# FeggieBoss/raytracing-course

Measured on NVIDIA B200. Metric: Mpaths/s, higher is better.
Workload: dtype f32

## Files before the change

include/rtc_b200.h:

```cpp
#ifndef RTC_B200_H
#define RTC_B200_H
#include <stdint.h>
#ifdef __cplusplus
extern "C" {
#endif

typedef struct rtc_scene rtc_scene;

typedef enum {
    RTC_OK = 0,
    RTC_ERR_IO = -1,
    RTC_ERR_NO_DEVICE = -2,
    RTC_ERR_CUDA = -3,
    RTC_ERR_ARG = -4,
    RTC_ERR_UNSUPPORTED = -5
} rtc_status;

#define RTC_TRAVERSAL_INDEX   0
#define RTC_TRAVERSAL_REFTREE 1

const char* rtc_last_error(void);
int rtc_version(void);
int rtc_device_count(void);

// ... 23 lines not shown
int rtc_intersect(const rtc_scene* s, long n, const float* o_host, const float* d_host,
                  int32_t* id_host, float* t_host, float* normal_host, int32_t* interior_host, int mode);
int rtc_intersect_dev(rtc_scene* s, long n, const float* o_dev, const float* d_dev, int32_t* id_dev, float* t_dev,
                      float* normal_dev, int32_t* interior_dev, int mode, void* stream);
int rtc_primitive_intersect(const rtc_scene* s, int prim, long n, const float* o_host, const float* d_host,
                            int32_t* hit_host, float* t_host, float* normal_host, int32_t* interior_host);
int rtc_camera_rays(const rtc_scene* s, long n, const float* xy_host, float* o_host, float* d_host);
int rtc_mix_pdf(const rtc_scene* s, long n, const float* x_host, const float* nrm_host, const float* d_host,
                float* pdf_host);
int rtc_mix_sample(const rtc_scene* s, long n, const float* x_host, const float* nrm_host,
                   uint32_t seed, uint32_t sample, uint32_t bounce, float* dir_host);
int rtc_tonemap_u8(const rtc_scene* s, long npix, const float* rgb_host, uint8_t* out_host);

int rtc_render_accumulate(rtc_scene* s, uint32_t seed, uint32_t sample_begin, uint32_t sample_count,
                          float* accum_dev, void* stream);
int rtc_render_counters(rtc_scene* s, void* stream, uint64_t out[8]);
int rtc_render_reset_counters(rtc_scene* s);
int rtc_traverse_lanes(rtc_scene* s, void* stream, uint64_t out[8]);
int rtc_render_resolve(rtc_scene* s, const float* accum_dev, uint32_t total_samples, uint8_t* rgb_dev, void* stream);
int rtc_render_u8(rtc_scene* s, uint32_t seed, uint8_t* rgb_host);
int rtc_render_sum(rtc_scene* s, uint32_t seed, uint32_t sample_begin, uint32_t sample_count, float* sum_host);
int rtc_render_ppm(rtc_scene* s, uint32_t seed, const char* out_path);
#define RTC_ADAPTIVE_TILE 8
int rtc_render_adaptive(rtc_scene* s, uint32_t seed, float tolerance, uint32_t min_samples, uint32_t max_samples,
                        uint8_t* rgb_host, float* halves_host, uint32_t* spp_host, uint64_t stats[4]);
int rtc_render_u8_multi(rtc_scene* s, const int* devices, int ndev, uint32_t seed, uint8_t* rgb_host, float* sum_host);
int rtc_render_ppm_multi(rtc_scene* s, const int* devices, int ndev, uint32_t seed, const char* out_path);
int rtc_render_adaptive_multi(rtc_scene* s, const int* devices, int ndev, uint32_t seed, float tolerance, uint32_t min_samples,
                              uint32_t max_samples, uint8_t* rgb_host, float* halves_host, uint32_t* spp_host, uint64_t stats[4]);
int rtc_denoise(rtc_scene* s, const float* halves_host, const uint32_t* spp_host, float strength, uint8_t* rgb_host, float* mean_host);
int rtc_render_denoised(rtc_scene* s, uint32_t seed, float tolerance, uint32_t min_samples, uint32_t max_samples, float strength,
// ... 20 lines not shown
```

raytracing-course_b200/__init__.py:

```python
import ctypes as C
import os

import numpy as np

HERE = os.path.dirname(os.path.abspath(__file__))
LIB_PATH = os.path.join(HERE, "librtc_b200.so")
CLI_PATH = os.path.join(HERE, "raytracing_hw5")
HEADER_PATH = os.path.join(os.path.dirname(HERE), "include", "rtc_b200.h")

TRAVERSAL_INDEX = 0
TRAVERSAL_REFTREE = 1
DENOISE_STRENGTH = 0.45

_f32 = np.ctypeslib.ndpointer(dtype=np.float32, flags="C_CONTIGUOUS")
_i32 = np.ctypeslib.ndpointer(dtype=np.int32, flags="C_CONTIGUOUS")
_u32 = np.ctypeslib.ndpointer(dtype=np.uint32, flags="C_CONTIGUOUS")
_u64 = np.ctypeslib.ndpointer(dtype=np.uint64, flags="C_CONTIGUOUS")
_u8 = np.ctypeslib.ndpointer(dtype=np.uint8, flags="C_CONTIGUOUS")

_SIGNATURES = {
    "rtc_last_error": (C.c_char_p, []),
    "rtc_version": (C.c_int, []),
    "rtc_device_count": (C.c_int, []),
    "rtc_scene_load": (C.c_void_p, [C.c_char_p, C.c_int]),
# ... 345 lines not shown
                                                    C.c_void_p(t_ptr), C.c_void_p(normal_ptr), C.c_void_p(interior_ptr),
                                                    mode, C.c_void_p(stream or 0)))

    def RenderPPM(self, path, seed=0):
        _check(self.lib, self.lib.rtc_render_ppm(self.h, seed, os.fsencode(path)))

    def render_accumulate(self, accum_ptr, seed, sample_begin, sample_count, stream=None):
        _check(self.lib, self.lib.rtc_render_accumulate(self.h, seed, sample_begin, sample_count,
                                                         C.c_void_p(accum_ptr), C.c_void_p(stream or 0)))

    def render_resolve(self, accum_ptr, total_samples, rgb_ptr, stream=None):
        _check(self.lib, self.lib.rtc_render_resolve(self.h, C.c_void_p(accum_ptr), total_samples,
                                                      C.c_void_p(rgb_ptr), C.c_void_p(stream or 0)))

    def counters(self, stream=None):
        out = np.zeros(8, np.uint64)
        _check(self.lib, self.lib.rtc_render_counters(self.h, C.c_void_p(stream or 0), out))
        keys = ["paths", "rays", "launches", "batches", "index_node_visits", "fallback_rays", "prim_tests", "traversed_rays"]
        return dict(zip(keys, [int(v) for v in out[:8]]))

    def traverse_lanes(self, stream=None):
        out = np.zeros(8, np.uint64)
        _check(self.lib, self.lib.rtc_traverse_lanes(self.h, C.c_void_p(stream or 0), out))
        kinds = ["visit", "leaf", "finish", "refill"]
        return {k: {"iterations": int(out[i]), "lanes": (float(out[4 + i]) / float(out[i]) if out[i] else 0.0)}
                for i, k in enumerate(kinds)}

    def set_profiling(self, kernel_events=False, count_visits=False):
        _check(self.lib, self.lib.rtc_set_profiling(self.h, int(kernel_events), int(count_visits)))

    def profile(self, stream=None, reset=True):
        ms = np.zeros(4, np.float64)
        n = np.zeros(4, np.uint64)
        _check(self.lib, self.lib.rtc_render_profile(self.h, C.c_void_p(stream or 0), ms, n, int(reset)))
# ... 18 lines not shown
```

raytracing-course_b200/csrc/bvh_build.cpp:

```cpp
#include <algorithm>
#include <chrono>
#include <cstdio>
#include <cstdlib>
#include <cmath>
#include <cstring>
#include <future>
#include <thread>
#include <numeric>
#include <stdexcept>

#include "scene_host.h"

namespace rtc {

static const float kInf = 1e18f;

static Aabb empty_box() { return Aabb{{kInf, kInf, kInf}, {-kInf, -kInf, -kInf}}; }
static void grow(Aabb& b, vec3 p) {
    b.mx.x = std::max(b.mx.x, p.x); b.mn.x = std::min(b.mn.x, p.x);
    b.mx.y = std::max(b.mx.y, p.y); b.mn.y = std::min(b.mn.y, p.y);
    b.mx.z = std::max(b.mx.z, p.z); b.mn.z = std::min(b.mn.z, p.z);
}
static void grow(Aabb& b, const Aabb& o) { grow(b, o.mx); grow(b, o.mn); }
static float surface(const Aabb& b) {
// ... 444 lines not shown
    std::memcpy(&r.w, &bits, 4);
    return r;
}

namespace {
struct PhaseTimer {
    bool on = std::getenv("RTC_TIMING") != nullptr;
    std::chrono::steady_clock::time_point t0 = std::chrono::steady_clock::now();
    void lap(const char* what) {
        if (!on) return;
        auto t1 = std::chrono::steady_clock::now();
        std::fprintf(stderr, "[rtc timing] %-28s %8.1f ms\n", what, std::chrono::duration<double, std::milli>(t1 - t0).count());
        t0 = t1;
    }
};
}

void HostScene::init() {
    PhaseTimer timer;
    const uint32_t n = (uint32_t)prims.size();
    if (n >= IREF_MAX_PRIMS) throw std::runtime_error("scene has more than 2^24 primitives");

    std::vector<Primitive> original = prims;
    std::vector<int32_t> perm(n);
    std::iota(perm.begin(), perm.end(), 0);
    const Primitive* P = original.data();
    nbvh = (uint32_t)(std::partition(perm.begin(), perm.end(), [P](int32_t i) { return P[i].type != PT_PLANE; }) - perm.begin());

    nodes.clear();
    root = 0;
// ... 33 lines not shown
            vec3 nrm = normalize(cross(p.d1 - p.d0, p.d2 - p.d0));
            F.geo0[i] = f4{p.d0.x, p.d0.y, p.d0.z, nrm.x};
            F.geo1[i] = f4{p.d1.x, p.d1.y, p.d1.z, nrm.y};
            F.geo2[i] = f4{p.d2.x, p.d2.y, p.d2.z, nrm.z};
        } else {
            F.geo0[i] = f4{p.d0.x, p.d0.y, p.d0.z, 0.f};
            F.geo1[i] = f4{0, 0, 0, 0};
            F.geo2[i] = f4{0, 0, 0, 0};
        }
        F.xf_pos[i] = pack(p.pos, flags);
        F.xf_rot[i] = f4{p.rot.x, p.rot.y, p.rot.z, p.rot.w};
        F.mat0[i] = pack(p.col, (uint32_t)p.material);
        F.mat1[i] = f4{p.emission.x, p.emission.y, p.emission.z, p.ior};
    }
    F.lights = lights;
    for (const PointLight& l : point_lights) {
        vec3 nd = l.directed ? normalize(l.dir) : mk3(0, 0, 0);
        F.plights.push_back(pack(l.intensity, l.directed ? 1u : 0u));
        F.plights.push_back(pack(l.pos, 0));
        F.plights.push_back(pack(l.att, 0));
        F.plights.push_back(pack(nd, 0));
    }
    for (uint32_t i = nbvh; i < n; ++i) {
        const Primitive& p = prims[i];
        bool rot_ident = p.rot.x == 0.f && p.rot.y == 0.f && p.rot.z == 0.f && p.rot.w == 1.f;
        F.planes.push_back(pack(p.d0, i));
        F.planes.push_back(pack(p.pos, rot_ident ? 1u : 0u));
    }

    timer.lap("flatten primitives");
// ... 88 lines not shown
```

raytracing-course_b200/csrc/c_api.cu:

```cuda
#include <cuda_runtime.h>

#include <algorithm>
#include <array>
#include <cfloat>
#include <cmath>
#include <chrono>
#include <cstdio>
#include <cstdlib>
#include <cstring>
#include <fstream>
#include <functional>
#include <map>
#include <memory>
#include <sstream>
#include <stdexcept>
#include <string>
#include <thread>
#include <vector>

#include "device_scene.h"
#include "rt_kernels.h"
#include "rtc_b200.h"
#include "scene_host.h"

// ... 42 lines not shown
    Handle() = default;
    Handle(Handle&& o) noexcept : h(o.h) { o.h = nullptr; }
    ~Handle() { if (h) destroy(h); }
    cudaError_t ensure() { return h ? cudaSuccess : create(&h); }
    operator H() const { return h; }
};
cudaError_t new_stream(cudaStream_t* st) { return cudaStreamCreateWithFlags(st, cudaStreamNonBlocking); }
cudaError_t new_event(cudaEvent_t* e) { return cudaEventCreateWithFlags(e, cudaEventDisableTiming); }
cudaError_t new_timed_event(cudaEvent_t* e) { return cudaEventCreate(e); }
using Stream = Handle<cudaStream_t, new_stream, cudaStreamDestroy>;
using Event = Handle<cudaEvent_t, new_event, cudaEventDestroy>;
using TimedEvent = Handle<cudaEvent_t, new_timed_event, cudaEventDestroy>;

constexpr uint64_t kDefaultBatchPaths = 1ull << 24;
constexpr int kMaxDepthSlots = 64;
constexpr int kStatWords = 16;
constexpr int kMaxWhittedDepth = 32;
}

struct rtc_scene {
    std::shared_ptr<HostScene> host_ptr;
    HostScene& host;
    rtc_scene() : host_ptr(std::make_shared<HostScene>()), host(*host_ptr) {}
    explicit rtc_scene(const std::shared_ptr<HostScene>& h) : host_ptr(h), host(*h) {}
    int device = -1;
    int sms = 0;
    int traversal = RTC_TRAVERSAL_INDEX;
    uint64_t batch_paths = kDefaultBatchPaths;
    uint64_t device_bytes = 0;
    DevBuf<unsigned char> arena_dev[2];
    PinnedBuf<unsigned char> arena_host;
// ... 420 lines not shown
        if (l.stream) {
            cudaError_t e = cudaStreamSynchronize(l.stream);
            if (e != cudaSuccess) return e;
        }
    return cudaSuccess;
}

int ensure_wavefront(rtc_scene* s, uint64_t cap, int nlanes) {
    for (int i = 0; i < nlanes; ++i) {
        rtc_scene::Lane& l = s->lanes[i];
        CU(l.stream.ensure());
        CU(l.done.ensure());
        for (auto& set : l.path) for (auto& b : set) CU(b.ensure(cap));
        for (auto& b : l.hit_id) CU(b.ensure(cap));
        CU(l.trav_queue.ensure(cap * kTraverseQueueWords));
        CU(l.queue.ensure(4 * kMaxDepthSlots));
    }
    return RTC_OK;
}

struct PathMap {
    const uint32_t* plist;
    uint32_t npix;
    uint32_t sample_first;
};
int fork_lanes(rtc_scene* s, cudaStream_t user) {
    CU(s->fork.ensure());
    CU(cudaEventRecord(s->fork, user));
    return RTC_OK;
}
int join_lanes(rtc_scene* s, unsigned used, cudaStream_t user) {
// ... 17 lines not shown
    const int nlanes = s->profiling ? 1 : whole ? s->nlanes : (int)(nbatches < (uint64_t)s->nlanes ? nbatches : (uint64_t)s->nlanes);
    const int lane_first = whole ? (int)(s->next_lane++ % (unsigned)s->nlanes) : 0;
    if ((rc = ensure_wavefront(s, cap, nlanes))) return rc;
    for (int i = 0; i < nlanes; ++i)
        if (!whole || i == lane_first) {
            CU(cudaStreamWaitEvent(s->lanes[i].stream, s->fork, 0));
            *used |= 1u << i;
        }
    uint64_t batch = 0;
    for (uint64_t first = 0; first < total; first += cap, ++batch) {
        rtc_scene::Lane& L = s->lanes[(lane_first + batch) % nlanes];
        cudaStream_t st = L.stream;
        LaunchCtx c{st, s->sms};
        uint32_t* tqc = L.queue.p + 2 * kMaxDepthSlots;
        uint32_t* cursor = L.queue.p + 3 * kMaxDepthSlots;
        uint32_t count = (uint32_t)((total - first) < cap ? (total - first) : cap);
        CU(cudaMemsetAsync(L.queue.p, 0, 4 * kMaxDepthSlots * sizeof(uint32_t), st));
        PathSoA cur{L.path[0][0].p, L.path[0][1].p, L.path[0][2].p};
        PathSoA nxt{L.path[1][0].p, L.path[1][1].p, L.path[1][2].p};
        HitSoA hcur{L.hit_id[0].p}, hnxt{L.hit_id[1].p};
        s->span_begin(0, st);
        if (map.plist) launch_generate_list(c, S, cur, hcur, L.queue.p, L.trav_queue.p, tqc, first, count, seed, map.plist, map.npix, map.sample_first);
        else launch_generate(c, S, cur, hcur, L.queue.p, L.trav_queue.p, tqc, first, count, seed, map.sample_first);
        s->span_end(st);
        s->launches++;
        for (uint32_t b = 1; b <= depth; ++b) {
            s->span_begin(1, st);
            if (s->traversal == RTC_TRAVERSAL_REFTREE) launch_extend_reftree(c, S, cur, hcur, L.queue.p + 2 * (b - 1), count);
            else launch_traverse(c, S, cur, hcur, count, L.trav_queue.p, tqc + (b - 1), cursor + (b - 1), s->count_visits, s->stats.p);
            s->span_end(st);
            s->span_begin(2, st);
            launch_shade(c, S, cur, hcur, nxt, hnxt, L.queue.p + 2 * (b - 1), L.queue.p + 2 * b, L.trav_queue.p, tqc + b, count,
                         target, b, seed);
            s->span_end(st);
            s->launches += 2;
            PathSoA tmp = cur; cur = nxt; nxt = tmp;
            HitSoA htmp = hcur; hcur = hnxt; hnxt = htmp;
        }
        launch_tally(c, L.queue.p, tqc, depth, s->stats.p);
        s->launches++;
    }
    return RTC_OK;
}

}

extern "C" {

const char* rtc_last_error(void) { return g_error.c_str(); }
int rtc_version(void) { return 100; }
int rtc_device_count(void) {
    int n = 0;
    if (cudaGetDeviceCount(&n) != cudaSuccess) { cudaGetLastError(); return 0; }
    return n;
// ... 279 lines not shown
    CU(accum4.ensure(npix));
    CU(cudaStreamWaitEvent(user, s->accum4_idle[a4], 0));
    CU(cudaMemsetAsync(accum4.p, 0, npix * sizeof(float4), user));
    if ((rc = arena_begin(s, user, &S))) return rc;
    if ((rc = fork_lanes(s, user))) return rc;
    unsigned used = 0;
    if ((rc = render_paths(s, S, seed, PathMap{nullptr, (uint32_t)npix, sample_begin}, total, accum4.p, &used))) return rc;
    if ((rc = join_lanes(s, used, user))) return rc;
    launch_fold(LaunchCtx{user, s->sms}, accum4.p, accum_dev, (uint32_t)npix);
    s->launches++;
    CU(cudaEventRecord(s->accum4_idle[a4], user));
    if ((rc = arena_end(s, user))) return rc;
    CU(cudaGetLastError());
    return RTC_OK;
}
int rtc_render_counters(rtc_scene* s, void* stream, uint64_t out[8]) {
    int rc = need_device(s);
    if (rc) return rc;
    if (!out) return fail(RTC_ERR_ARG, "null argument");
    CU(cudaStreamSynchronize((cudaStream_t)stream));
    CU(sync_lanes(s));
    unsigned long long h[8];
    CU(cudaMemcpy(h, s->stats.p, sizeof h, cudaMemcpyDeviceToHost));
    for (int i = 0; i < 8; ++i) out[i] = h[i];
    out[2] = s->launches;
    return RTC_OK;
}
int rtc_traverse_lanes(rtc_scene* s, void* stream, uint64_t out[8]) {
    int rc = need_device(s);
    if (rc) return rc;
    if (!out) return fail(RTC_ERR_ARG, "null argument");
    CU(cudaStreamSynchronize((cudaStream_t)stream));
    CU(sync_lanes(s));
    unsigned long long h[8];
    CU(cudaMemcpy(h, s->stats.p + 8, sizeof h, cudaMemcpyDeviceToHost));
    for (int i = 0; i < 8; ++i) out[i] = h[i];
    return RTC_OK;
}
int rtc_render_reset_counters(rtc_scene* s) {
    int rc = need_device(s);
// ... 672 lines not shown
```

raytracing-course_b200/csrc/device_scene.h:

```cpp
#pragma once
#include <cuda_runtime.h>
#include <math.h>
#include <stdint.h>
#include <string.h>

#include "scene_host.h"

namespace rtc {

struct DevScene {
    const float4* geo0;
    const float4* geo1;
    const float4* geo2;
    const float4* xf_pos;
    const float4* xf_rot;
    const float4* mat0;
    const float4* mat1;
    const float4* inodes;
    const float4* rnodes;
    const uint4* rmeta;
    const uint32_t* lca;
    const int32_t* lights;
    const float4* ubox;
    const float4* planes;
    const float4* plights;

    uint32_t nprims, nbvh, nnodes, root, iroot, lca_levels, nlights, ref_depth;
    uint32_t iroot_ref[4];
    uint32_t width, height, ray_depth, nplanes;
    float3 cam_pos, cam_right, cam_up, cam_forward;
    float tan_fov_x, tan_fov_y;
    float3 bg;
    uint32_t dialect, nplights;
    uint32_t features;
    float eps;
    float plane_tmax;
    float3 ambient;
};

inline void fill_dev_scalars(const HostScene& host, DevScene& S) {
    S.nplanes = (uint32_t)(host.flat.planes.size() / 2);
    S.nprims = (uint32_t)host.prims.size(); S.nbvh = host.nbvh; S.nnodes = (uint32_t)host.nodes.size();
    S.root = host.root; S.iroot = host.flat.iroot; S.lca_levels = host.flat.lca_levels;
    for (int c = 0; c < 4; ++c) S.iroot_ref[c] = IREF_NONE;
    if (host.flat.iroot != IREF_NONE && !(host.flat.iroot & IREF_LEAF)) {
        const f4& refs = host.flat.inodes[kIndexNodeF4 * (size_t)(host.flat.iroot & IREF_NODE_MASK) + 3];
        memcpy(S.iroot_ref, &refs, sizeof S.iroot_ref);
    }
    S.nlights = (uint32_t)host.lights.size(); S.ref_depth = host.flat.ref_depth;
    S.width = host.cam.width; S.height = host.cam.height; S.ray_depth = host.ray_depth;
    S.cam_pos = make_float3(host.cam.pos.x, host.cam.pos.y, host.cam.pos.z);
    S.cam_right = make_float3(host.cam.right.x, host.cam.right.y, host.cam.right.z);
    S.cam_up = make_float3(host.cam.up.x, host.cam.up.y, host.cam.up.z);
    S.cam_forward = make_float3(host.cam.forward.x, host.cam.forward.y, host.cam.forward.z);
    float tx = (float)tan((double)(host.cam.fov_x / 2));
    S.tan_fov_x = tx;
    S.tan_fov_y = tx * (float)host.cam.height / (float)host.cam.width;
    S.bg = make_float3(host.background.x, host.background.y, host.background.z);
    S.nplights = (uint32_t)host.point_lights.size();
    S.dialect = (uint32_t)host.dialect;
    S.features = host.flat.features;
    S.eps = host.dialect <= DIALECT_HW3 ? 1e-3f : 1e-4f;
    S.plane_tmax = host.dialect <= DIALECT_HW3 ? 3.0e38f : 1e5f;
    S.ambient = make_float3(host.ambient.x, host.ambient.y, host.ambient.z);
}

struct PathSoA {
    float4* o;
    float4* d;
    float4* beta;
};
struct HitSoA {
    uint32_t* id;
};

constexpr uint32_t HIT_MISS = 0xFFFFFFFFu;
constexpr uint32_t HIT_INTERIOR = 1u << 30;

}
// ... 1 lines not shown
```

raytracing-course_b200/csrc/rt_device.cuh:

```cuda
#pragma once
#include <cuda_fp16.h>
#include <cuda_runtime.h>
#include <math_constants.h>
#include <stdint.h>

#include "device_scene.h"
#include "scene_host.h"
#include "vecmath.h"

namespace rtc {

#define RT_D __device__ __forceinline__
#ifdef __CUDACC__
#define RT_D_COLD static __device__ __noinline__
#else
#define RT_D_COLD static inline
#endif

constexpr float kInfF = 1e18f;
constexpr float kPi = 3.14159274101257324f;
constexpr int kRejectCap = 64;
constexpr int kMaxRecords = 24;
constexpr int kIndexStack = 64;
constexpr int kRefStack = 96;
// ... 583 lines not shown
        if (!(FEAT & FE_ROTATION) || __float_as_uint(b.w)) {
            vec3 n = ld3(a);
            t = -dot(o - ld3(b), n) / dot(d, n);
            ok = t > 0.f && !(t > S.plane_tmax);
        } else {
            vec3 lo = o, ld = d;
            to_local(S, prim, prim_flags(S, prim), lo, ld);
            Isect is;
            ok = isect_plane(lo, ld, ld3(a), S.plane_tmax, is);
            t = is.t;
        }
        if (ok && t < closest) { closest = t; id = (int)prim; }
    }
}

struct SceneHit {
    int id;
    float t;
    vec3 n;
    int interior;
};

template <int MODE>
RT_D SceneHit scene_intersect(const DevScene& S, vec3 o, vec3 d, uint32_t* visits, uint32_t* tests, uint32_t* fallbacks) {
    SceneHit h;
    h.id = -1; h.t = 0.f; h.n = mk3(0, 0, 0); h.interior = 0;
    float closest;
    closest_plane(S, o, d, closest, h.id);
    BestHit b;
    if (MODE == 1) {
// ... 188 lines not shown
```

raytracing-course_b200/csrc/rt_kernels.cu:

```cuda
#include <cassert>

#include "rt_device.cuh"
#include "rt_kernels.h"

namespace rtc {

static_assert(kNodeWidth == 4, "a traverse-queue entry carries the 4 root children a ray enters");
constexpr unsigned kFullMask = 0xFFFFFFFFu;
#ifndef RTC_TRAVERSE_CHUNK
#define RTC_TRAVERSE_CHUNK 64
#endif
#ifndef RTC_TRAVERSE_CHUNK_DIV
#define RTC_TRAVERSE_CHUNK_DIV 4
#endif
#ifndef RTC_TRAVERSE_CHUNK_MAX
#define RTC_TRAVERSE_CHUNK_MAX 512
#endif
constexpr uint32_t kChunk = RTC_TRAVERSE_CHUNK;

#ifndef RTC_NO_STREAM_STATE
#define WF_LD(ptr) __ldcs(ptr)
#define WF_ST(ptr, v) __stcs(ptr, v)
#else
#define WF_LD(ptr) (*(ptr))
// ... 323 lines not shown
#endif
}

#ifndef RTC_SHADE_THREADS
#define RTC_SHADE_THREADS 128
#endif
#ifndef RTC_SHADE_MIN_BLOCKS_FULL
#define RTC_SHADE_MIN_BLOCKS_FULL 6
#endif
#ifndef RTC_SHADE_MIN_BLOCKS_LEAN
#define RTC_SHADE_MIN_BLOCKS_LEAN 9
#endif
template <bool HW3, uint32_t FEAT>
__global__ void __launch_bounds__(RTC_SHADE_THREADS, (FEAT & (FE_ROTATION | FE_ELLIPSOID)) ? RTC_SHADE_MIN_BLOCKS_FULL : RTC_SHADE_MIN_BLOCKS_LEAN) k_shade(DevScene S, PathSoA P, HitSoA H, PathSoA N, HitSoA HN, const uint32_t* qin,
                                                uint32_t* qout, uint32_t* tq, uint32_t* tq_count, float4* accum4, uint32_t bounce,
                                                uint32_t seed, uint32_t cap) {
    const QueueView view = queue_view(qin);
    const uint32_t lane = threadIdx.x & 31;
    const float eps = S.eps;
    const bool sorted_in = bounce > 1 && !HW3;
    const bool sort_out = !HW3 && S.nlights != 0 && bounce + 1 < S.ray_depth;
    for (uint32_t at = blockIdx.x * blockDim.x + threadIdx.x; at < view.total; at += gridDim.x * blockDim.x) {
        bool alive = false;
        vec3 no = mk3(0, 0, 0), nd = mk3(0, 0, 0), beta = mk3(0, 0, 0);
        uint32_t pixel = 0, sample = 0;
        uint32_t i; bool back;
        if (queue_slot(view, at, cap, i, back)) {
            const float4 b4 = WF_LD(P.beta + i), o4 = WF_LD(P.o + i);
            beta = ld3(b4);
            pixel = __float_as_uint(b4.w); sample = __float_as_uint(o4.w);
            uint32_t prim = WF_LD(H.id + i);
            Isect is;
            vec3 o = ld3(o4), d = ld3(WF_LD(P.d + i));
            vec3 L;
            float4 xp = make_float4(0.f, 0.f, 0.f, 0.f), g0 = xp, g1 = xp, g2 = xp, m0 = xp, m1 = xp;
            if (prim != HIT_MISS) {
// ... 57 lines not shown
                            vec3 rd = reflect_dir(normal, nd_in);
                            no = p + eps * rd; nd = rd;
                        } else {
                            float cos2 = sqrtf(1.f - sin2 * sin2);
                            float e = eta1 / eta2;
                            vec3 fr = e * (-dir) + (e * dn - cos2) * normal;
                            no = p + eps * fr; nd = fr;
                            if (!interior) beta = beta * col;
                        }
                        alive = true;
                    }
                }
            }
            if (L.x != 0.f || L.y != 0.f || L.z != 0.f) deposit(accum4, pixel, L);
        }
        unsigned mask = __ballot_sync(kFullMask, alive);
        if (mask) {
            const uint32_t lt = (1u << lane) - 1u;
            bool to_back = false;
            if (sort_out && alive) to_back = mix_picks_light(S, Rng{seed, pixel, sample, bounce + 1});
            const unsigned bmask = __ballot_sync(kFullMask, to_back), fmask = mask & ~bmask;
            unsigned long long both = 0;
            uint32_t tbase = 0;
            if (lane == 0) both = atomicAdd(reinterpret_cast<unsigned long long*>(qout),
                                            (unsigned long long)__popc(fmask) | ((unsigned long long)__popc(bmask) << 32));
            float cd = 0.f;
            uint32_t id = HIT_MISS, enters = 0;
            if (alive) enters = pre_step<FEAT>(S, no, nd, cd, id);
            const unsigned emask = __ballot_sync(kFullMask, enters != 0);
            if (emask && lane == 0) tbase = atomicAdd(tq_count, (uint32_t)__popc(emask));
            both = __shfl_sync(kFullMask, both, 0);
            const uint32_t dst = to_back ? cap - 1u - ((uint32_t)(both >> 32) + __popc(bmask & lt))
                                         : (uint32_t)both + __popc(fmask & lt);
            if (alive) {
                WF_ST(N.o + dst, make_float4(no.x, no.y, no.z, __uint_as_float(sample)));
                WF_ST(N.d + dst, make_float4(nd.x, nd.y, nd.z, cd));
                WF_ST(N.beta + dst, make_float4(beta.x, beta.y, beta.z, __uint_as_float(pixel)));
                WF_ST(HN.id + dst, id);
            }
            if (emask) {
                tbase = __shfl_sync(kFullMask, tbase, 0);
                if (enters) tq_store(tq, tbase + __popc(emask & lt), dst | (enters << kTqSlotBits), no, nd, cd);
            }
        }
    }
}

__global__ void k_tally(const uint32_t* q, const uint32_t* tqc, uint32_t ray_depth, unsigned long long* stats) {
    unsigned long long rays = 0, queued = 0;
    for (uint32_t b = 0; b < ray_depth; ++b) { rays += q[2 * b] + q[2 * b + 1]; queued += tqc[b]; }
    atomicAdd(stats + 0, (unsigned long long)q[0]);
    atomicAdd(stats + 1, rays);
    atomicAdd(stats + 3, 1ull);
    atomicAdd(stats + 7, queued);
}

RT_D float aces(float x) {
    const float a = 2.51f, b = 0.03f, c = 2.43f, d = 0.59f, e = 0.14f;
    float num = __fmul_rn(x, __fadd_rn(__fmul_rn(a, x), b));
    float den = __fadd_rn(__fmul_rn(x, __fadd_rn(__fmul_rn(c, x), d)), e);
    float y = __fdiv_rn(num, den);
    y = (y < 1.f) ? y : 1.f;
    y = (y < 0.f) ? 0.f : y;
    return y;
}
// ... 385 lines not shown
    }
    return cache[slot][dev];
}
void launch_traverse(const LaunchCtx& c, const DevScene& S, PathSoA P, HitSoA H, uint32_t max_count, const uint32_t* tq,
                     const uint32_t* tq_count, uint32_t* cursor, bool count_visits, unsigned long long* stats) {
    const int per_sm = count_visits ? resident_blocks(k_traverse<true>, 1) : resident_blocks(k_traverse<false>, 0);
    int grid = grid_for((uint64_t)max_count, 128, c.sms, per_sm);
    if (count_visits) k_traverse<true><<<grid, 128, 0, c.stream>>>(S, P, H, tq, tq_count, cursor, stats);
    else k_traverse<false><<<grid, 128, 0, c.stream>>>(S, P, H, tq, tq_count, cursor, stats);
}
void launch_extend_reftree(const LaunchCtx& c, const DevScene& S, PathSoA P, HitSoA H, const uint32_t* q, uint32_t cap) {
    k_extend_reftree<<<grid_for(cap, 128, c.sms, 16), 128, 0, c.stream>>>(S, P, H, q, cap);
}
void launch_shade(const LaunchCtx& c, const DevScene& S, PathSoA P, HitSoA H, PathSoA N, HitSoA HN, const uint32_t* qin,
                  uint32_t* qout, uint32_t* tq, uint32_t* tq_count, uint32_t max_count, float4* accum4, uint32_t bounce,
                  uint32_t seed) {
    const int grid = grid_for(max_count, RTC_SHADE_THREADS, c.sms, 2048 / RTC_SHADE_THREADS);
#define RTC_SHADE(HW3, FEAT) k_shade<HW3, FEAT><<<grid, RTC_SHADE_THREADS, 0, c.stream>>>(S, P, H, N, HN, qin, qout, tq, tq_count, accum4, bounce, seed, max_count)
#ifdef RTC_SHADE_NO_SPECIALISATION
    const uint32_t feat = FE_ALL;
#else
    const uint32_t feat = S.features;
#endif
    if (S.dialect == DIALECT_HW3) RTC_SHADE(true, FE_ALL);
    else if (feat == 0) RTC_SHADE(false, 0);
    else if (feat == FE_SPECULAR) RTC_SHADE(false, FE_SPECULAR);
    else RTC_SHADE(false, FE_ALL);
#undef RTC_SHADE
}
void launch_expand_lca(const LaunchCtx& c, uint32_t* lca, const uint4* rmeta, uint32_t n, uint32_t levels) {
    for (uint32_t l = 1; l < levels; ++l)
        k_expand_lca_level<<<grid_for(n, 256, c.sms, 8), 256, 0, c.stream>>>(lca + (size_t)(l - 1) * n, lca + (size_t)l * n, rmeta, n, 1u << (l - 1));
}
void launch_expand_boxes(const LaunchCtx& c, const float4* sparse, uint32_t n, float4* ubox) {
    k_expand_boxes<<<grid_for(n, 256, c.sms, 8), 256, 0, c.stream>>>(sparse, n, ubox);
}
void launch_expand_palette(const LaunchCtx& c, const float4* palette, const uint16_t* index, uint32_t n, float4* out0, float4* out1) {
    k_expand_palette<<<grid_for(n, 256, c.sms, 8), 256, 0, c.stream>>>(palette, index, n, out0, out1);
}
void launch_fill_identity_rotations(const LaunchCtx& c, float4* rot, uint32_t n) {
    k_fill_identity_rotations<<<grid_for(n, 256, c.sms, 8), 256, 0, c.stream>>>(rot, n);
}
void launch_tally(const LaunchCtx& c, const uint32_t* q, const uint32_t* tqc, uint32_t ray_depth, unsigned long long* stats) {
    k_tally<<<1, 1, 0, c.stream>>>(q, tqc, ray_depth, stats);
}
void launch_fold(const LaunchCtx& c, const float4* accum4, float* accum, uint32_t npix) {
    k_fold<<<grid_for(npix, 256, c.sms, 8), 256, 0, c.stream>>>(accum4, accum, npix);
}
void launch_resolve(const LaunchCtx& c, const float* accum, float inv_samples, uint32_t nvalues, uint8_t* out) {
    k_resolve<<<grid_for(nvalues, 256, c.sms, 8), 256, 0, c.stream>>>(accum, inv_samples, nvalues, out);
}
void launch_resolve_peers(const LaunchCtx& c, const PeerAccums& A, float inv_samples, uint32_t nvalues, uint8_t* out, float* sum) {
    k_resolve_peers<<<grid_for(nvalues, 256, c.sms, 8), 256, 0, c.stream>>>(A, inv_samples, nvalues, out, sum);
}
void launch_tonemap(const LaunchCtx& c, const float* rgb, uint32_t nvalues, uint8_t* out) {
    k_tonemap<<<grid_for(nvalues, 256, c.sms, 8), 256, 0, c.stream>>>(rgb, nvalues, out);
}
void launch_pack_rays(const LaunchCtx& c, long n, const float* o, const float* d, PathSoA P, uint32_t* q) {
    k_pack_rays<<<grid_for((uint64_t)n, 256, c.sms, 8), 256, 0, c.stream>>>(n, o, d, P, q);
// ... 22 lines not shown
```

raytracing-course_b200/csrc/rt_kernels.h:

```cpp
#pragma once
#include <cuda_runtime.h>
#include <stdint.h>

#include "device_scene.h"

namespace rtc {

constexpr uint32_t kTraverseQueueWords = 8;

struct LaunchCtx {
    cudaStream_t stream;
    int sms;
};

void launch_generate(const LaunchCtx& c, const DevScene& S, PathSoA P, HitSoA H, uint32_t* q, uint32_t* tq, uint32_t* tq_count,
                     uint64_t first_path, uint32_t count, uint32_t seed, uint32_t sample_begin);
void launch_generate_list(const LaunchCtx& c, const DevScene& S, PathSoA P, HitSoA H, uint32_t* q, uint32_t* tq, uint32_t* tq_count,
                          uint64_t first_path, uint32_t count, uint32_t seed, const uint32_t* plist, uint32_t npix, uint32_t sample_first);
constexpr uint32_t kAdaptiveTile = 8;
static_assert(kAdaptiveTile * kAdaptiveTile == 64, "k_adaptive_tiles: one warp per tile, two pixels per lane");
enum { ADAPTIVE_FIRST = 0, ADAPTIVE_DECIDE = 1, ADAPTIVE_LAST = 2 };
void launch_adaptive_tiles(const LaunchCtx& c, const float4* A, const float4* B, uint32_t width, uint32_t height,
                           const uint32_t* tiles_in, uint32_t ntiles, uint32_t n, float inv_a, float inv_b, float tau, int mode,
                           uint32_t* tile_n, uint32_t* tiles_out, uint32_t* pixels_out, uint32_t* counts_out, uint32_t shard,
// ... 3 lines not shown
constexpr int kDenoiseRadius = 7, kDenoisePatch = 3, kDenoiseVarRadius = 1;
constexpr float kDenoiseAlpha = 1.f, kDenoiseEps = 1e-8f;
constexpr int kDenoiseTileW = 32, kDenoiseTileH = 16;
constexpr int kDenoiseApron = kDenoiseRadius + kDenoisePatch + kDenoiseVarRadius;
void launch_denoise_prep(const LaunchCtx& c, const float* halves, const uint32_t* spp, uint32_t npix, float* u, float4* D, float4* V,
                         uint8_t* rgb);
cudaError_t launch_denoise_nlm(const LaunchCtx& c, const float* u, const float4* D, const float4* V, uint32_t width, uint32_t height,
                               uint32_t tile_row0, uint32_t tile_rows, uint32_t buf_row0, float k2, float* mean, uint8_t* rgb);
void launch_pre(const LaunchCtx& c, const DevScene& S, PathSoA P, HitSoA H, const uint32_t* qcount, uint32_t max_count,
                uint32_t* tq, uint32_t* tq_count);
void launch_traverse(const LaunchCtx& c, const DevScene& S, PathSoA P, HitSoA H, uint32_t max_count, const uint32_t* tq,
                     const uint32_t* tq_count, uint32_t* cursor, bool count_visits, unsigned long long* stats);
void launch_extend_reftree(const LaunchCtx& c, const DevScene& S, PathSoA P, HitSoA H, const uint32_t* q, uint32_t cap);
void launch_shade(const LaunchCtx& c, const DevScene& S, PathSoA P, HitSoA H, PathSoA N, HitSoA HN, const uint32_t* qin,
                  uint32_t* qout, uint32_t* tq, uint32_t* tq_count, uint32_t max_count, float4* accum4, uint32_t bounce,
                  uint32_t seed);
void launch_fold(const LaunchCtx& c, const float4* accum4, float* accum, uint32_t npix);
void launch_expand_lca(const LaunchCtx& c, uint32_t* lca, const uint4* rmeta, uint32_t n, uint32_t levels);
void launch_expand_boxes(const LaunchCtx& c, const float4* sparse, uint32_t n, float4* ubox);
void launch_fill_identity_rotations(const LaunchCtx& c, float4* rot, uint32_t n);
void launch_expand_palette(const LaunchCtx& c, const float4* palette, const uint16_t* index, uint32_t n, float4* out0, float4* out1);
void launch_tally(const LaunchCtx& c, const uint32_t* q, const uint32_t* tqc, uint32_t ray_depth, unsigned long long* stats);
void launch_resolve(const LaunchCtx& c, const float* accum, float inv_samples, uint32_t nvalues, uint8_t* out);
void launch_tonemap(const LaunchCtx& c, const float* rgb, uint32_t nvalues, uint8_t* out);
constexpr int kMaxPeers = 16;
struct PeerAccums {
    const float* p[kMaxPeers];
    int n;
};
void launch_resolve_peers(const LaunchCtx& c, const PeerAccums& A, float inv_samples, uint32_t nvalues, uint8_t* out, float* sum);
struct PeerHalves {
    const float4* a[kMaxPeers];
    const float4* b[kMaxPeers];
    const uint32_t* tile_n[kMaxPeers];
    int n;
};
void launch_resolve_adaptive_peers(const LaunchCtx& c, const PeerHalves& P, uint32_t width, uint32_t npix, uint8_t* out, float* halves,
// ... 19 lines not shown
```

raytracing-course_b200/csrc/scene_host.h:

```cpp
#pragma once
#include <cstdint>
#include <string>
#include <vector>

#include "vecmath.h"

#ifndef RTC_NODE_CONES
#define RTC_NODE_CONES 1
#endif
#ifndef RTC_NODE_CENTRE_HALF
#define RTC_NODE_CENTRE_HALF 1
#endif

namespace rtc {

enum Dialect : int {
    DIALECT_HW1 = 1,
    DIALECT_HW2 = 2,
    DIALECT_HW3 = 3,
    DIALECT_HW4 = 4,
    DIALECT_HW5 = 5
};

struct PointLight {
// ... 54 lines not shown
    std::vector<f4> xf_pos;
    std::vector<f4> xf_rot;
    std::vector<f4> mat0, mat1;
    std::vector<f4> inodes;
    uint32_t iroot = 0;
    std::vector<f4> rnodes;
    std::vector<u4> rmeta;
    std::vector<uint32_t> lca;
    uint32_t lca_levels = 0;
    std::vector<f4> ubox;
    std::vector<f4> planes;
    std::vector<int32_t> lights;
    std::vector<f4> plights;
    uint32_t index_depth = 0, ref_depth = 0, units = 0;
    uint32_t features = 0;
};

struct HostScene {
    int dialect = DIALECT_HW5;
    Camera cam;
    vec3 background{0, 0, 0};
    vec3 ambient{0, 0, 0};
    std::vector<PointLight> point_lights;
    unsigned ray_depth = 0, samples = 0;
    std::vector<Primitive> prims;
    uint32_t nbvh = 0;
    std::vector<RefNode> nodes;
    uint32_t root = 0;
    std::vector<int32_t> lights;
    FlatScene flat;

// ... 23 lines not shown
```

Before: 2047.

## Retire final-bounce rays that cannot reach emitters and early-miss rays in shade

Computes conservative world-space AABBs for emissive boxes and ellipsoids on the host and stores them in the device scene. On the last bounce, the shade kernel drops rays whose direction misses every emitter box, since they cannot add radiance. Rays that pre_step already shows miss the scene are resolved in place with the background contribution and never reach the traversal queue. New counters track retired rays. This saves traversal and shading work in exchange for extra per-ray box tests and an added atomic per warp; scenes with other emitter types or more than eight emitters turn the final-bounce cull off.

```diff
diff --git a/include/rtc_b200.h b/include/rtc_b200.h
--- a/include/rtc_b200.h
+++ b/include/rtc_b200.h
@@ -61,7 +61,7 @@
 
 int rtc_render_accumulate(rtc_scene* s, uint32_t seed, uint32_t sample_begin, uint32_t sample_count,
                           float* accum_dev, void* stream);
-int rtc_render_counters(rtc_scene* s, void* stream, uint64_t out[8]);
+int rtc_render_counters(rtc_scene* s, void* stream, uint64_t out[10]);
 int rtc_render_reset_counters(rtc_scene* s);
 int rtc_traverse_lanes(rtc_scene* s, void* stream, uint64_t out[8]);
 int rtc_render_resolve(rtc_scene* s, const float* accum_dev, uint32_t total_samples, uint8_t* rgb_dev, void* stream);
diff --git a/raytracing-course_b200/__init__.py b/raytracing-course_b200/__init__.py
--- a/raytracing-course_b200/__init__.py
+++ b/raytracing-course_b200/__init__.py
@@ -383,10 +383,11 @@
                                                       C.c_void_p(rgb_ptr), C.c_void_p(stream or 0)))
 
     def counters(self, stream=None):
-        out = np.zeros(8, np.uint64)
+        out = np.zeros(10, np.uint64)
         _check(self.lib, self.lib.rtc_render_counters(self.h, C.c_void_p(stream or 0), out))
-        keys = ["paths", "rays", "launches", "batches", "index_node_visits", "fallback_rays", "prim_tests", "traversed_rays"]
-        return dict(zip(keys, [int(v) for v in out[:8]]))
+        keys = ["paths", "rays", "launches", "batches", "index_node_visits", "fallback_rays", "prim_tests", "traversed_rays",
+                "retired_rays", "retired_final_rays"]
+        return dict(zip(keys, [int(v) for v in out]))
 
     def traverse_lanes(self, stream=None):
         out = np.zeros(8, np.uint64)
diff --git a/raytracing-course_b200/csrc/bvh_build.cpp b/raytracing-course_b200/csrc/bvh_build.cpp
--- a/raytracing-course_b200/csrc/bvh_build.cpp
+++ b/raytracing-course_b200/csrc/bvh_build.cpp
@@ -482,6 +482,55 @@
         t0 = t1;
     }
 };
+bool emitter_boxes(const HostScene& h, std::vector<f4>& out) {
+    out.clear();
+    double extent = std::max({std::fabs((double)h.cam.pos.x), std::fabs((double)h.cam.pos.y), std::fabs((double)h.cam.pos.z)});
+    if (h.nbvh) {
+        const Aabb& r = h.nodes[h.root].box;
+        extent = std::max({extent, std::fabs((double)r.mn.x), std::fabs((double)r.mn.y), std::fabs((double)r.mn.z),
+                           std::fabs((double)r.mx.x), std::fabs((double)r.mx.y), std::fabs((double)r.mx.z)});
+    }
+    for (const Primitive& p : h.prims) {
+        if (p.emission.x == 0.f && p.emission.y == 0.f && p.emission.z == 0.f) continue;
+        if ((p.type != PT_BOX && p.type != PT_ELLIPSOID) || out.size() == 2 * kMaxEmitBoxes) { out.clear(); return false; }
+        const double qx = -(double)p.rot.x, qy = -(double)p.rot.y, qz = -(double)p.rot.z, qw = p.rot.w;
+        double M[3][3];
+        for (int c = 0; c < 3; ++c) {
+            const double v[3] = {c == 0 ? 1. : 0., c == 1 ? 1. : 0., c == 2 ? 1. : 0.};
+            const double u[3] = {qy * v[2] - qz * v[1], qz * v[0] - qx * v[2], qx * v[1] - qy * v[0]};
+            const double uu[3] = {qy * u[2] - qz * u[1], qz * u[0] - qx * u[2], qx * u[1] - qy * u[0]};
+            for (int r = 0; r < 3; ++r) M[r][c] = v[r] + 2. * (qw * u[r] + uu[r]);
+        }
+        const double det = M[0][0] * (M[1][1] * M[2][2] - M[1][2] * M[2][1]) - M[0][1] * (M[1][0] * M[2][2] - M[1][2] * M[2][0]) +
+                           M[0][2] * (M[1][0] * M[2][1] - M[1][1] * M[2][0]);
+        if (!(std::fabs(det) > 1e-9)) { out.clear(); return false; }
+        double I[3][3];
+        for (int r = 0; r < 3; ++r)
+            for (int c = 0; c < 3; ++c) {
+                const int r1 = (c + 1) % 3, r2 = (c + 2) % 3, c1 = (r + 1) % 3, c2 = (r + 2) % 3;
+                I[r][c] = (M[r1][c1] * M[r2][c2] - M[r1][c2] * M[r2][c1]) / det;
+            }
+        double lo[3] = {INFINITY, INFINITY, INFINITY}, hi[3] = {-INFINITY, -INFINITY, -INFINITY};
+        const double s[3] = {p.d0.x, p.d0.y, p.d0.z}, pos[3] = {p.pos.x, p.pos.y, p.pos.z};
+        for (int corner = 0; corner < 8; ++corner)
+            for (int r = 0; r < 3; ++r) {
+                double w = pos[r];
+                for (int c = 0; c < 3; ++c) w += I[r][c] * ((corner >> c & 1) ? s[c] : -s[c]);
+                lo[r] = std::min(lo[r], w);
+                hi[r] = std::max(hi[r], w);
+            }
+        float flo[3], fhi[3];
+        for (int r = 0; r < 3; ++r) {
+            const double pad = 1e-3 * std::max({extent, std::fabs(lo[r]), std::fabs(hi[r])});
+            flo[r] = std::nextafter((float)(lo[r] - pad), -INFINITY);
+            fhi[r] = std::nextafter((float)(hi[r] + pad), INFINITY);
+            if (!std::isfinite(flo[r]) || !std::isfinite(fhi[r])) { out.clear(); return false; }
+        }
+        out.push_back(f4{flo[0], flo[1], flo[2], 0.f});
+        out.push_back(f4{fhi[0], fhi[1], fhi[2], 0.f});
+    }
+    return true;
+}
 }
 
 void HostScene::init() {
@@ -545,6 +594,7 @@
         F.mat1[i] = f4{p.emission.x, p.emission.y, p.emission.z, p.ior};
     }
     F.lights = lights;
+    F.final_cull = emitter_boxes(*this, F.emit_boxes);
     for (const PointLight& l : point_lights) {
         vec3 nd = l.directed ? normalize(l.dir) : mk3(0, 0, 0);
         F.plights.push_back(pack(l.intensity, l.directed ? 1u : 0u));
diff --git a/raytracing-course_b200/csrc/c_api.cu b/raytracing-course_b200/csrc/c_api.cu
--- a/raytracing-course_b200/csrc/c_api.cu
+++ b/raytracing-course_b200/csrc/c_api.cu
@@ -80,7 +80,7 @@
 
 constexpr uint64_t kDefaultBatchPaths = 1ull << 24;
 constexpr int kMaxDepthSlots = 64;
-constexpr int kStatWords = 16;
+constexpr int kStatWords = 18;
 constexpr int kMaxWhittedDepth = 32;
 }
 
@@ -531,7 +531,7 @@
         for (auto& set : l.path) for (auto& b : set) CU(b.ensure(cap));
         for (auto& b : l.hit_id) CU(b.ensure(cap));
         CU(l.trav_queue.ensure(cap * kTraverseQueueWords));
-        CU(l.queue.ensure(4 * kMaxDepthSlots));
+        CU(l.queue.ensure(6 * kMaxDepthSlots));
     }
     return RTC_OK;
 }
@@ -579,8 +579,9 @@
         LaunchCtx c{st, s->sms};
         uint32_t* tqc = L.queue.p + 2 * kMaxDepthSlots;
         uint32_t* cursor = L.queue.p + 3 * kMaxDepthSlots;
+        unsigned long long* retired = reinterpret_cast<unsigned long long*>(L.queue.p + 4 * kMaxDepthSlots);
         uint32_t count = (uint32_t)((total - first) < cap ? (total - first) : cap);
-        CU(cudaMemsetAsync(L.queue.p, 0, 4 * kMaxDepthSlots * sizeof(uint32_t), st));
+        CU(cudaMemsetAsync(L.queue.p, 0, 6 * kMaxDepthSlots * sizeof(uint32_t), st));
         PathSoA cur{L.path[0][0].p, L.path[0][1].p, L.path[0][2].p};
         PathSoA nxt{L.path[1][0].p, L.path[1][1].p, L.path[1][2].p};
         HitSoA hcur{L.hit_id[0].p}, hnxt{L.hit_id[1].p};
@@ -596,13 +597,13 @@
             s->span_end(st);
             s->span_begin(2, st);
             launch_shade(c, S, cur, hcur, nxt, hnxt, L.queue.p + 2 * (b - 1), L.queue.p + 2 * b, L.trav_queue.p, tqc + b, count,
-                         target, b, seed);
+                         target, b, seed, retired + b);
             s->span_end(st);
             s->launches += 2;
             PathSoA tmp = cur; cur = nxt; nxt = tmp;
             HitSoA htmp = hcur; hcur = hnxt; hnxt = htmp;
         }
-        launch_tally(c, L.queue.p, tqc, depth, s->stats.p);
+        launch_tally(c, L.queue.p, tqc, retired, depth, s->stats.p);
         s->launches++;
     }
     return RTC_OK;
@@ -912,16 +913,18 @@
     CU(cudaGetLastError());
     return RTC_OK;
 }
-int rtc_render_counters(rtc_scene* s, void* stream, uint64_t out[8]) {
+int rtc_render_counters(rtc_scene* s, void* stream, uint64_t out[10]) {
     int rc = need_device(s);
     if (rc) return rc;
     if (!out) return fail(RTC_ERR_ARG, "null argument");
     CU(cudaStreamSynchronize((cudaStream_t)stream));
     CU(sync_lanes(s));
-    unsigned long long h[8];
+    unsigned long long h[kStatWords];
     CU(cudaMemcpy(h, s->stats.p, sizeof h, cudaMemcpyDeviceToHost));
     for (int i = 0; i < 8; ++i) out[i] = h[i];
     out[2] = s->launches;
+    out[8] = h[16];
+    out[9] = h[17];
     return RTC_OK;
 }
 int rtc_traverse_lanes(rtc_scene* s, void* stream, uint64_t out[8]) {
diff --git a/raytracing-course_b200/csrc/device_scene.h b/raytracing-course_b200/csrc/device_scene.h
--- a/raytracing-course_b200/csrc/device_scene.h
+++ b/raytracing-course_b200/csrc/device_scene.h
@@ -36,6 +36,8 @@
     float eps;
     float plane_tmax;
     float3 ambient;
+    uint32_t final_cull, nemit;
+    float3 emit_lo[kMaxEmitBoxes], emit_hi[kMaxEmitBoxes];
 };
 
 inline void fill_dev_scalars(const HostScene& host, DevScene& S) {
@@ -63,6 +65,14 @@
     S.eps = host.dialect <= DIALECT_HW3 ? 1e-3f : 1e-4f;
     S.plane_tmax = host.dialect <= DIALECT_HW3 ? 3.0e38f : 1e5f;
     S.ambient = make_float3(host.ambient.x, host.ambient.y, host.ambient.z);
+    S.final_cull = host.flat.final_cull ? 1u : 0u;
+    S.nemit = (uint32_t)(host.flat.emit_boxes.size() / 2);
+    for (uint32_t i = 0; i < kMaxEmitBoxes; ++i) {
+        const bool on = i < S.nemit;
+        const f4 lo = on ? host.flat.emit_boxes[2 * i] : f4{0, 0, 0, 0}, hi = on ? host.flat.emit_boxes[2 * i + 1] : f4{0, 0, 0, 0};
+        S.emit_lo[i] = make_float3(lo.x, lo.y, lo.z);
+        S.emit_hi[i] = make_float3(hi.x, hi.y, hi.z);
+    }
 }
 
 struct PathSoA {
diff --git a/raytracing-course_b200/csrc/rt_device.cuh b/raytracing-course_b200/csrc/rt_device.cuh
--- a/raytracing-course_b200/csrc/rt_device.cuh
+++ b/raytracing-course_b200/csrc/rt_device.cuh
@@ -621,6 +621,21 @@
     }
 }
 
+RT_D bool emitter_reachable(const DevScene& S, vec3 o, vec3 d) {
+    const vec3 inv = mk3(__fdividef(1.f, d.x), __fdividef(1.f, d.y), __fdividef(1.f, d.z));
+    bool reach = false;
+    for (uint32_t i = 0; i < S.nemit; ++i) {
+        const float ax = (S.emit_lo[i].x - o.x) * inv.x, bx = (S.emit_hi[i].x - o.x) * inv.x;
+        const float ay = (S.emit_lo[i].y - o.y) * inv.y, by = (S.emit_hi[i].y - o.y) * inv.y;
+        const float az = (S.emit_lo[i].z - o.z) * inv.z, bz = (S.emit_hi[i].z - o.z) * inv.z;
+        const float t1 = fmaxf(fmaxf(fminf(ax, bx), fminf(ay, by)), fminf(az, bz));
+        const float t2 = fminf(fminf(fmaxf(ax, bx), fmaxf(ay, by)), fmaxf(az, bz));
+        const bool nan = ax != ax || bx != bx || ay != ay || by != by || az != az || bz != bz;
+        reach = reach || nan || (t1 <= t2 && t2 >= 0.f);
+    }
+    return reach;
+}
+
 struct SceneHit {
     int id;
     float t;
diff --git a/raytracing-course_b200/csrc/rt_kernels.cu b/raytracing-course_b200/csrc/rt_kernels.cu
--- a/raytracing-course_b200/csrc/rt_kernels.cu
+++ b/raytracing-course_b200/csrc/rt_kernels.cu
@@ -361,12 +361,14 @@
 template <bool HW3, uint32_t FEAT>
 __global__ void __launch_bounds__(RTC_SHADE_THREADS, (FEAT & (FE_ROTATION | FE_ELLIPSOID)) ? RTC_SHADE_MIN_BLOCKS_FULL : RTC_SHADE_MIN_BLOCKS_LEAN) k_shade(DevScene S, PathSoA P, HitSoA H, PathSoA N, HitSoA HN, const uint32_t* qin,
                                                 uint32_t* qout, uint32_t* tq, uint32_t* tq_count, float4* accum4, uint32_t bounce,
-                                                uint32_t seed, uint32_t cap) {
+                                                uint32_t seed, uint32_t cap, unsigned long long* retired) {
     const QueueView view = queue_view(qin);
     const uint32_t lane = threadIdx.x & 31;
     const float eps = S.eps;
     const bool sorted_in = bounce > 1 && !HW3;
     const bool sort_out = !HW3 && S.nlights != 0 && bounce + 1 < S.ray_depth;
+    const bool cull_final = S.final_cull && bounce + 1 == S.ray_depth;
+    const bool bg_zero = S.bg.x == 0.f && S.bg.y == 0.f && S.bg.z == 0.f;
     for (uint32_t at = blockIdx.x * blockDim.x + threadIdx.x; at < view.total; at += gridDim.x * blockDim.x) {
         bool alive = false;
         vec3 no = mk3(0, 0, 0), nd = mk3(0, 0, 0), beta = mk3(0, 0, 0);
@@ -454,6 +456,23 @@
             }
             if (L.x != 0.f || L.y != 0.f || L.z != 0.f) deposit(accum4, pixel, L);
         }
+        bool retire_final = false;
+        if (cull_final && alive)
+            retire_final = isfinite(beta.x) && isfinite(beta.y) && isfinite(beta.z) && !emitter_reachable(S, no, nd);
+        float cd = 0.f;
+        uint32_t id = HIT_MISS, enters = 0;
+        if (alive && !(retire_final && bg_zero)) enters = pre_step<FEAT>(S, no, nd, cd, id);
+        retire_final = retire_final && cd < kInfF;
+        const bool retire_miss = alive && !retire_final && enters == 0 && id == HIT_MISS;
+        if (retire_miss) {
+            const vec3 Lb = beta * mk3(S.bg.x, S.bg.y, S.bg.z);
+            if (Lb.x != 0.f || Lb.y != 0.f || Lb.z != 0.f) deposit(accum4, pixel, Lb);
+        }
+        const unsigned rfmask = __ballot_sync(kFullMask, retire_final), rmmask = __ballot_sync(kFullMask, retire_miss);
+        if ((rfmask | rmmask) && lane == 0)
+            atomicAdd(retired, (unsigned long long)__popc(rmmask) | ((unsigned long long)__popc(rfmask) << 32));
+        alive = alive && !retire_final && !retire_miss;
+        if (!alive) enters = 0;
         unsigned mask = __ballot_sync(kFullMask, alive);
         if (mask) {
             const uint32_t lt = (1u << lane) - 1u;
@@ -464,9 +483,6 @@
             uint32_t tbase = 0;
             if (lane == 0) both = atomicAdd(reinterpret_cast<unsigned long long*>(qout),
                                             (unsigned long long)__popc(fmask) | ((unsigned long long)__popc(bmask) << 32));
-            float cd = 0.f;
-            uint32_t id = HIT_MISS, enters = 0;
-            if (alive) enters = pre_step<FEAT>(S, no, nd, cd, id);
             const unsigned emask = __ballot_sync(kFullMask, enters != 0);
             if (emask && lane == 0) tbase = atomicAdd(tq_count, (uint32_t)__popc(emask));
             both = __shfl_sync(kFullMask, both, 0);
@@ -486,9 +502,18 @@
     }
 }
 
-__global__ void k_tally(const uint32_t* q, const uint32_t* tqc, uint32_t ray_depth, unsigned long long* stats) {
-    unsigned long long rays = 0, queued = 0;
-    for (uint32_t b = 0; b < ray_depth; ++b) { rays += q[2 * b] + q[2 * b + 1]; queued += tqc[b]; }
+__global__ void k_tally(const uint32_t* q, const uint32_t* tqc, const unsigned long long* retired, uint32_t ray_depth,
+                        unsigned long long* stats) {
+    unsigned long long rays = 0, queued = 0, retired_miss = 0, retired_final = 0;
+    for (uint32_t b = 0; b < ray_depth; ++b) {
+        rays += q[2 * b] + q[2 * b + 1];
+        queued += tqc[b];
+        retired_miss += retired[b] & 0xFFFFFFFFull;
+        retired_final += retired[b] >> 32;
+    }
+    rays += retired_miss + retired_final;
+    atomicAdd(stats + 16, retired_miss + retired_final);
+    atomicAdd(stats + 17, retired_final);
     atomicAdd(stats + 0, (unsigned long long)q[0]);
     atomicAdd(stats + 1, rays);
     atomicAdd(stats + 3, 1ull);
@@ -904,9 +929,9 @@
 }
 void launch_shade(const LaunchCtx& c, const DevScene& S, PathSoA P, HitSoA H, PathSoA N, HitSoA HN, const uint32_t* qin,
                   uint32_t* qout, uint32_t* tq, uint32_t* tq_count, uint32_t max_count, float4* accum4, uint32_t bounce,
-                  uint32_t seed) {
+                  uint32_t seed, unsigned long long* retired) {
     const int grid = grid_for(max_count, RTC_SHADE_THREADS, c.sms, 2048 / RTC_SHADE_THREADS);
-#define RTC_SHADE(HW3, FEAT) k_shade<HW3, FEAT><<<grid, RTC_SHADE_THREADS, 0, c.stream>>>(S, P, H, N, HN, qin, qout, tq, tq_count, accum4, bounce, seed, max_count)
+#define RTC_SHADE(HW3, FEAT) k_shade<HW3, FEAT><<<grid, RTC_SHADE_THREADS, 0, c.stream>>>(S, P, H, N, HN, qin, qout, tq, tq_count, accum4, bounce, seed, max_count, retired)
 #ifdef RTC_SHADE_NO_SPECIALISATION
     const uint32_t feat = FE_ALL;
 #else
@@ -931,8 +956,9 @@
 void launch_fill_identity_rotations(const LaunchCtx& c, float4* rot, uint32_t n) {
     k_fill_identity_rotations<<<grid_for(n, 256, c.sms, 8), 256, 0, c.stream>>>(rot, n);
 }
-void launch_tally(const LaunchCtx& c, const uint32_t* q, const uint32_t* tqc, uint32_t ray_depth, unsigned long long* stats) {
-    k_tally<<<1, 1, 0, c.stream>>>(q, tqc, ray_depth, stats);
+void launch_tally(const LaunchCtx& c, const uint32_t* q, const uint32_t* tqc, const unsigned long long* retired, uint32_t ray_depth,
+                  unsigned long long* stats) {
+    k_tally<<<1, 1, 0, c.stream>>>(q, tqc, retired, ray_depth, stats);
 }
 void launch_fold(const LaunchCtx& c, const float4* accum4, float* accum, uint32_t npix) {
     k_fold<<<grid_for(npix, 256, c.sms, 8), 256, 0, c.stream>>>(accum4, accum, npix);
diff --git a/raytracing-course_b200/csrc/rt_kernels.h b/raytracing-course_b200/csrc/rt_kernels.h
--- a/raytracing-course_b200/csrc/rt_kernels.h
+++ b/raytracing-course_b200/csrc/rt_kernels.h
@@ -41,13 +41,14 @@
 void launch_extend_reftree(const LaunchCtx& c, const DevScene& S, PathSoA P, HitSoA H, const uint32_t* q, uint32_t cap);
 void launch_shade(const LaunchCtx& c, const DevScene& S, PathSoA P, HitSoA H, PathSoA N, HitSoA HN, const uint32_t* qin,
                   uint32_t* qout, uint32_t* tq, uint32_t* tq_count, uint32_t max_count, float4* accum4, uint32_t bounce,
-                  uint32_t seed);
+                  uint32_t seed, unsigned long long* retired);
 void launch_fold(const LaunchCtx& c, const float4* accum4, float* accum, uint32_t npix);
 void launch_expand_lca(const LaunchCtx& c, uint32_t* lca, const uint4* rmeta, uint32_t n, uint32_t levels);
 void launch_expand_boxes(const LaunchCtx& c, const float4* sparse, uint32_t n, float4* ubox);
 void launch_fill_identity_rotations(const LaunchCtx& c, float4* rot, uint32_t n);
 void launch_expand_palette(const LaunchCtx& c, const float4* palette, const uint16_t* index, uint32_t n, float4* out0, float4* out1);
-void launch_tally(const LaunchCtx& c, const uint32_t* q, const uint32_t* tqc, uint32_t ray_depth, unsigned long long* stats);
+void launch_tally(const LaunchCtx& c, const uint32_t* q, const uint32_t* tqc, const unsigned long long* retired, uint32_t ray_depth,
+                  unsigned long long* stats);
 void launch_resolve(const LaunchCtx& c, const float* accum, float inv_samples, uint32_t nvalues, uint8_t* out);
 void launch_tonemap(const LaunchCtx& c, const float* rgb, uint32_t nvalues, uint8_t* out);
 constexpr int kMaxPeers = 16;
diff --git a/raytracing-course_b200/csrc/scene_host.h b/raytracing-course_b200/csrc/scene_host.h
--- a/raytracing-course_b200/csrc/scene_host.h
+++ b/raytracing-course_b200/csrc/scene_host.h
@@ -92,7 +92,10 @@
     std::vector<f4> plights;
     uint32_t index_depth = 0, ref_depth = 0, units = 0;
     uint32_t features = 0;
+    std::vector<f4> emit_boxes;
+    bool final_cull = false;
 };
+constexpr uint32_t kMaxEmitBoxes = 8;
 
 struct HostScene {
     int dialect = DIALECT_HW5;
```

Result: slower. 2019 (median of 6 runs) (-1.4%).
